# kmaninis/OSVOS-PyTorch

Hardware: NVIDIA H100
Metric: frames/sec at 480x854 fwd-only, batch 1 per GPU (OSVOS.forward -> 5 logit maps) (higher is better)
Workload: dtype bf16x3 (split-bf16 operands, fp32 accumulate)

## Files before the change

include/osvos_b200.h:

```cpp
#ifndef OSVOS_B200_H_
#define OSVOS_B200_H_

#include <stddef.h>
#include <stdint.h>

#ifdef __cplusplus
extern "C" {
#endif

#define OSVOS_B200_VERSION 100

#if defined(__GNUC__)
#define OSVOS_API __attribute__((visibility("default")))
#else
#define OSVOS_API
#endif

enum {
  OSVOS_OK = 0,
  OSVOS_ERR_INVALID_ARGUMENT = 1,
  OSVOS_ERR_CUDA = 2,
  OSVOS_ERR_UNSUPPORTED = 3
};

// ... 30 lines not shown
  const void* x_lo;
  const void* w_packed;
  const float* bias;
  void* y_hi;
  void* y_lo;
  float* y_f32;
  const void* mask_hi;
  const float* proj_w;
  const float* proj_b;
  float* pq;
  void* pool_hi;
  void* pool_lo;
  float* colsum;
  int n, h, w, cin, cout;
  int flags;
} osvos_conv3x3_args;
OSVOS_API int osvos_conv3x3(const osvos_conv3x3_args* args , osvos_stream_t stream);

OSVOS_API int osvos_side_folded_multi(const osvos_conv3x3_args* args , int count, osvos_stream_t stream);

typedef struct {
  const float* side_w;
  const float* side_b;
  const float* proj_w;
  const float* proj_b;
  void* packed;
  float* bias2;
  float* folded_f32;
  int cin;
} osvos_fold_item;
OSVOS_API int osvos_fold_side_weights_multi(const osvos_fold_item* items , int count, osvos_stream_t stream);
OSVOS_API int osvos_conv3x3_simt(const osvos_conv3x3_args* args , osvos_stream_t stream);

typedef struct {
// ... 332 lines not shown
```

osvos_pytorch_b200/_native.py:

```python
import ctypes
import os
from ctypes import (POINTER, Structure, c_char_p, c_double, c_float, c_int, c_int32, c_size_t, c_uint8, c_uint32,
                    c_uint64, c_void_p)

_HERE = os.path.dirname(os.path.abspath(__file__))
LIB_PATH = os.path.join(_HERE, "lib", "libosvos_b200.so")

FLAG_RELU = 1
FLAG_FAST = 2
FLAG_RELU_MASK = 4
FLAG_ACCUMULATE = 8
FLAG_DEFER_FINISH = 16
FLAG_DETERMINISTIC = 32
FLAG_VOID_LABELS = 64
WGRAD_FINISH_MAX = 24


class NativeLibraryError(RuntimeError):
    pass


class Conv3x3Args(Structure):
    _fields_ = [("x_hi", c_void_p), ("x_lo", c_void_p), ("w_packed", c_void_p), ("bias", c_void_p),
                ("y_hi", c_void_p), ("y_lo", c_void_p), ("y_f32", c_void_p), ("mask_hi", c_void_p),
                ("proj_w", c_void_p), ("proj_b", c_void_p), ("pq", c_void_p),
                ("pool_hi", c_void_p), ("pool_lo", c_void_p), ("colsum", c_void_p),
                ("n", c_int), ("h", c_int), ("w", c_int), ("cin", c_int), ("cout", c_int), ("flags", c_int)]


class Stage1Args(Structure):
    _fields_ = [("x", c_void_p), ("w1", c_void_p), ("b1", c_void_p), ("w2_packed", c_void_p), ("b2", c_void_p),
                ("y_hi", c_void_p), ("y_lo", c_void_p), ("pool_hi", c_void_p), ("pool_lo", c_void_p),
                ("n", c_int), ("h", c_int), ("w", c_int)]


class TailFwdArgs(Structure):
    _fields_ = [("pq", c_void_p * 4), ("fuse_bias", c_void_p), ("out", c_void_p * 5), ("label", c_void_p),
                ("sums", c_void_p), ("losses", c_void_p), ("loss_weights", c_float * 5), ("divisor", c_float),
                ("n", c_int), ("h", c_int), ("w", c_int), ("flags", c_int)]


TAIL_SUMS = 15
# ... 2 lines not shown
class TailLossBwdArgs(Structure):
    _fields_ = [("logits", c_void_p * 5), ("label", c_void_p), ("sums", c_void_p), ("upstream", c_void_p),
                ("loss_weights", c_float * 5), ("divisor", c_float), ("dpq", c_void_p * 4), ("fuse_bias_grad", c_void_p),
                ("n", c_int), ("h", c_int), ("w", c_int), ("flags", c_int)]


class WgradArgs(Structure):
    _fields_ = [("x_hi", c_void_p), ("x_lo", c_void_p), ("dz_hi", c_void_p), ("dz_lo", c_void_p), ("dw", c_void_p),
                ("workspace", c_void_p), ("n", c_int), ("h", c_int), ("w", c_int), ("cin", c_int), ("cout", c_int),
                ("dz_channels", c_int), ("flags", c_int)]


class WgradFinishItem(Structure):
    _fields_ = [("workspace", c_void_p), ("dw", c_void_p), ("cout", c_int), ("cin", c_int), ("dz_channels", c_int),
                ("accumulate", c_int), ("scale", c_float)]


class FoldItem(Structure):
    _fields_ = [("side_w", c_void_p), ("side_b", c_void_p), ("proj_w", c_void_p), ("proj_b", c_void_p),
                ("packed", c_void_p), ("bias2", c_void_p), ("folded_f32", c_void_p), ("cin", c_int)]


class SideWgradItem(Structure):
    _fields_ = [("x_hi", c_void_p), ("x_lo", c_void_p), ("dpq", c_void_p), ("g", c_void_p), ("n", c_int), ("h", c_int),
                ("w", c_int), ("c", c_int)]


class SideGradsItem(Structure):
    _fields_ = [("g", c_void_p), ("side_w", c_void_p), ("side_b", c_void_p), ("proj_w", c_void_p),
                ("d_side_w", c_void_p), ("d_side_b", c_void_p), ("d_score_w", c_void_p), ("d_score_b", c_void_p),
# ... 62 lines not shown
SGD_MAX_SEGMENTS = 64

SIGNATURES = {
    "osvos_version": (c_int, []),
    "osvos_last_error": (c_char_p, []),
    "osvos_packed_weight_bytes": (c_size_t, [c_int, c_int]),
    "osvos_pack_conv3x3_weights": (c_int, [c_void_p, c_void_p, c_int, c_int, c_int, c_int, c_void_p]),
    "osvos_nchw_to_act": (c_int, [c_void_p, c_void_p, c_void_p, c_int, c_int, c_int, c_int, c_void_p]),
    "osvos_act_to_nchw": (c_int, [c_void_p, c_void_p, c_void_p, c_int, c_int, c_int, c_int, c_void_p]),
    "osvos_conv_first_fwd": (c_int, [c_void_p, c_void_p, c_void_p, c_void_p, c_void_p, c_int, c_int, c_int, c_int,
                                     c_void_p]),
    "osvos_conv3x3": (c_int, [POINTER(Conv3x3Args), c_void_p]),
    "osvos_stage1_fused": (c_int, [POINTER(Stage1Args), c_void_p]),
    "osvos_set_pdl": (c_int, [c_int]),
    "osvos_side_folded_multi": (c_int, [POINTER(Conv3x3Args), c_int, c_void_p]),
    "osvos_fold_side_weights_multi": (c_int, [POINTER(FoldItem), c_int, c_void_p]),
    "osvos_conv3x3_simt": (c_int, [POINTER(Conv3x3Args), c_void_p]),
    "osvos_maxpool2x2_fwd": (c_int, [c_void_p, c_void_p, c_void_p, c_void_p, c_int, c_int, c_int, c_int, c_void_p]),
    "osvos_tail_fwd": (c_int, [POINTER(TailFwdArgs), c_void_p]),
    "osvos_cbce_fwd_sums": (c_size_t, [c_size_t, c_int]),
    "osvos_cbce_fwd": (c_int, [c_void_p, c_void_p, c_size_t, c_double, c_void_p, c_void_p, c_int, c_void_p]),
    "osvos_cbce_bwd": (c_int, [c_void_p, c_void_p, c_void_p, c_void_p, c_double, c_size_t, c_void_p, c_void_p]),
    "osvos_cbce_bwd_void": (c_int, [c_void_p, c_void_p, c_void_p, c_void_p, c_double, c_size_t, c_void_p, c_void_p]),
    "osvos_wgrad_workspace_bytes": (c_size_t, [c_int, c_int, c_int, c_int, c_int, c_int]),
    "osvos_conv3x3_wgrad": (c_int, [POINTER(WgradArgs), c_void_p]),
    "osvos_wgrad_finish": (c_int, [POINTER(WgradFinishItem), POINTER(c_int), c_int, c_int, c_void_p]),
    "osvos_tail_bwd": (c_int, [POINTER(TailBwdArgs), c_void_p]),
    "osvos_tail_loss_bwd": (c_int, [POINTER(TailLossBwdArgs), c_void_p]),
    "osvos_sum_f32_scratch_bytes": (c_size_t, [c_int]),
    "osvos_sum_f32": (c_int, [c_void_p, c_size_t, c_void_p, c_void_p, c_int, c_void_p]),
# ... 108 lines not shown
```

osvos_pytorch_b200/autograd.py:

```python
import torch

from . import ops


class _OSVOSFunction(torch.autograd.Function):
    @staticmethod
    def forward(ctx, engine, x, objective, *params):
        with ops.no_uninitialized_fill():
            return _OSVOSFunction._forward(ctx, engine, x, objective, *params)

    @staticmethod
    def backward(ctx, *grads):
        with ops.no_uninitialized_fill():
            return _OSVOSFunction._backward(ctx, *grads)

    @staticmethod
    def _forward(ctx, engine, x, objective, *params):
        m = engine.m
        fast = m.precision == "fast"
        general = engine.uses_general_tail()
        ctx.params = params
        ctx.set_materialize_grads(False)
        det = torch.are_deterministic_algorithms_enabled()
        ctx.det = det
        xin = x.detach().contiguous().float()
        n, _, h, w = (int(v) for v in xin.shape)
        acts, pooled = engine._trunk(xin, fast, keep=True)
        feats, pqs = engine._side_outputs([s[-1] for s in acts[1:]], fast)
        if general:
            table = engine._upsampling_table()
            ctx.general = (feats, pqs, table)

            def tail(**kw):
                return ops.tail_general_fwd(feats, pqs, table, m.fuse.bias.detach(), n, h, w, **kw)
        else:
            ctx.general = None

            def tail(**kw):
                return ops.tail_fwd(pqs, m.fuse.bias.detach(), n, h, w, **kw)
        ctx.engine = engine
        ctx.dims = (n, h, w)
        ctx.fast = fast
# ... 252 lines not shown
```

osvos_pytorch_b200/csrc/conv3x3_halo.cu:

```cuda
#include "conv_common.cuh"

namespace osvos {

constexpr int kHaloRows = kTileH + 2;
constexpr int kPitch = kTileW + 2;

template <int BLOCK_N, int PLANES, bool SPLIT>
struct HaloCfg {
  static constexpr int kABoxBytes = kHaloRows * kPitch * 128;
  static constexpr int kAPlaneBytes = (kABoxBytes + 1023) / 1024 * 1024;
  static constexpr int kAStageBytes = PLANES * kAPlaneBytes;
  static constexpr int kAStages = 2;
  static constexpr int kBPlaneBytes = BLOCK_N * 128;
  static constexpr int kBStageBytes = PLANES * kBPlaneBytes;
  static constexpr int kBudget = 225 * 1024 - kAStages * kAStageBytes;
  static constexpr int kBStagesRaw = kBudget / kBStageBytes;
  static constexpr int kBStages = kBStagesRaw > 9 ? 9 : kBStagesRaw;
  static constexpr bool kSplitAcc = SPLIT;
  static_assert(!SPLIT || (PLANES == 2 && BLOCK_N <= 128), "split accumulators need two planes and 2 * BLOCK_N <= 256");
  static constexpr int kAccCols = kSplitAcc ? 2 * BLOCK_N : BLOCK_N;
  static constexpr int kAcc = kAccCols / 2;
  static constexpr int kSmemBytes = kAStages * kAStageBytes + kBStages * kBStageBytes + 1024 + 512;
  static_assert(kBStages >= 2, "weight ring too shallow");
  static_assert(kSmemBytes <= 227 * 1024, "more than the per-CTA shared memory of sm_90");
// ... 167 lines not shown
          if (tap == 8) pending.bar_a = &a_empty[a_stage];
          if (++b_stage == SB) {
            b_stage = 0;
            b_phase ^= 1;
          }
        }
        if (++a_stage == SA) {
          a_stage = 0;
          a_phase ^= 1;
        }
      }
      wgmma_wait<0>();
#pragma unroll
      for (int h = 0; h < kHalves; ++h) wgmma_fence_operands(acc[h]);
      pending.release(leader);
#pragma unroll
      for (int h = 0; h < kHalves; ++h)
        conv_epilogue<BLOCK_N, Cfg::kSplitAcc, LEAN, DET>(p, acc[h], tile, PINGPONG ? h : wg, wl, lane);
    }
  }
}

template <int BLOCK_N, int PLANES, bool LEAN = false, bool DET = false>
static int launch_halo(const osvos_conv3x3_args* a, cudaStream_t stream) {
  constexpr bool kSplit = PLANES == 2 && BLOCK_N <= 128;
  using Cfg = HaloCfg<BLOCK_N, PLANES, kSplit>;
  ConvParams p;
  fill_conv_params(p, a, BLOCK_N);
  const int sms = device_sm_count();
  CUtensorMap mx_hi, mx_lo, mw_hi, mw_lo;
  {
    const uint64_t dims[4] = {(uint64_t)a->cin, (uint64_t)a->w, (uint64_t)a->h, (uint64_t)a->n};
    const uint64_t strides[3] = {(uint64_t)a->cin * 2, (uint64_t)a->w * a->cin * 2,
// ... 8 lines not shown
  }
  int rc = encode_weight_maps(&mw_hi, &mw_lo, a, BLOCK_N);
  if (rc) return rc;
  const int grid = p.total_tiles < sms ? p.total_tiles : sms;
  constexpr bool kCanPingPong = BLOCK_N == 64 || BLOCK_N == 128;
  const bool pingpong = kCanPingPong && p.total_tiles > 2 * sms;
  auto kern = pingpong ? conv3x3_halo_kernel<BLOCK_N, PLANES, kSplit && BLOCK_N == 64, LEAN, kCanPingPong, DET>
                       : conv3x3_halo_kernel<BLOCK_N, PLANES, kSplit, LEAN, false, DET>;
  static uint64_t attr_done[2] = {0, 0};
  OSVOS_CHECK_CUDA(ensure_dynamic_smem(kern, Cfg::kSmemBytes, &attr_done[pingpong]));
  OSVOS_CHECK_CUDA(launch_pdl(kern, dim3(grid), dim3(kConvThreads), Cfg::kSmemBytes, stream, mx_hi, mx_lo,
                              mw_hi, mw_lo, p));
  return OSVOS_OK;
}

template <bool DET>
static int conv3x3_halo_dispatch(const osvos_conv3x3_args* a, cudaStream_t stream) {
  const bool fast = (a->flags & OSVOS_FLAG_FAST) != 0;
  const bool lean = !fast && !(a->flags & OSVOS_FLAG_RELU_MASK) && a->colsum == nullptr && a->y_f32 == nullptr;
  const int m_tiles = ((a->w + kTileW - 1) / kTileW) * ((a->h + kTileH - 1) / kTileH) * a->n;
  const int sms = device_sm_count();
  const long tiles128 = static_cast<long>(m_tiles) * (a->cout / 128);
  const long waves128 = (tiles128 + sms - 1) / sms;
  const long waves256 = (static_cast<long>(m_tiles) * (a->cout / 256) + sms - 1) / sms;
  if (a->cout == 64 || (waves128 == 1 && tiles128 * 5 <= static_cast<long>(sms) * 3)) {
    if (lean) return launch_halo<64, 2, true>(a, stream);
    return fast ? launch_halo<64, 1, false, DET>(a, stream) : launch_halo<64, 2, false, DET>(a, stream);
  }
  if (fast) {
    const bool prefer256 = waves256 * 1100 < waves128 * 700;
    if (a->cout % 256 == 0 && prefer256) return launch_halo<256, 1, false, DET>(a, stream);
    return launch_halo<128, 1, false, DET>(a, stream);
  }
  if (lean) return launch_halo<128, 2, true>(a, stream);
  return launch_halo<128, 2, false, DET>(a, stream);
}

static int check_conv_args(const osvos_conv3x3_args* a) {
  OSVOS_CHECK_ARG(a != nullptr);
  OSVOS_CHECK_ARG(a->n > 0 && a->h > 0 && a->w > 0);
  OSVOS_CHECK_ARG(a->cin >= 64 && a->cin % 64 == 0);
  OSVOS_CHECK_ARG(a->cout == 2 || a->cout == 16 || a->cout == 64 || (a->cout > 0 && a->cout % 128 == 0));
  OSVOS_CHECK_ARG(a->cout != 2 || (a->pq != nullptr && a->y_hi == nullptr && a->y_f32 == nullptr && a->pool_hi == nullptr &&
                                   a->colsum == nullptr && !(a->flags & (OSVOS_FLAG_RELU | OSVOS_FLAG_RELU_MASK))));
  OSVOS_CHECK_ARG(a->cout != 16 || (a->y_hi == nullptr && a->y_lo == nullptr && !(a->flags & OSVOS_FLAG_RELU_MASK)));
  OSVOS_CHECK_ARG(a->x_hi != nullptr && a->w_packed != nullptr);
  OSVOS_CHECK_ARG((a->flags & OSVOS_FLAG_FAST) || a->x_lo != nullptr);
  OSVOS_CHECK_ARG(a->y_hi != nullptr || a->y_f32 != nullptr || a->pq != nullptr || a->pool_hi != nullptr);
  OSVOS_CHECK_ARG(!(a->flags & OSVOS_FLAG_RELU_MASK) || a->mask_hi != nullptr);
  OSVOS_CHECK_ARG(a->pq == nullptr || a->cout == 2 || (a->cout == 16 && a->proj_w != nullptr));
  OSVOS_CHECK_ARG((a->pool_hi == nullptr && a->colsum == nullptr) || a->cout >= 64);
  OSVOS_CHECK_ARG((reinterpret_cast<uintptr_t>(a->x_hi) & 15) == 0);
  OSVOS_CHECK_ARG((reinterpret_cast<uintptr_t>(a->w_packed) & 15) == 0);
  OSVOS_CHECK_ARG((reinterpret_cast<uintptr_t>(a->bias) & 15) == 0);
  OSVOS_CHECK_ARG(!(a->flags & OSVOS_FLAG_DETERMINISTIC) || (reinterpret_cast<uintptr_t>(a->colsum) & 7) == 0);
  if (a->cout >= 64) {
    const uintptr_t bf16_planes = reinterpret_cast<uintptr_t>(a->y_hi) | reinterpret_cast<uintptr_t>(a->y_lo) |
                                  reinterpret_cast<uintptr_t>(a->pool_hi) | reinterpret_cast<uintptr_t>(a->pool_lo) |
                                  reinterpret_cast<uintptr_t>(a->mask_hi);
    OSVOS_CHECK_ARG((bf16_planes & 3) == 0);
    OSVOS_CHECK_ARG((reinterpret_cast<uintptr_t>(a->y_f32) & 7) == 0);
  }
  return OSVOS_OK;
}

}
// ... 16 lines not shown
      order[j] = order[j - 1];
      order[j - 1] = t;
    }
  return side_conv_multi_dispatch(order, count, static_cast<cudaStream_t>(stream_));
}

extern "C" int osvos_conv3x3(const osvos_conv3x3_args* a, osvos_stream_t stream_) {
  int rc = check_conv_args(a);
  if (rc) return rc;
  cudaStream_t stream = static_cast<cudaStream_t>(stream_);
  if (a->cout == 2 || a->cout == 16) return side_conv_dispatch(a, stream);
  if ((a->flags & OSVOS_FLAG_DETERMINISTIC) && a->colsum != nullptr) return conv3x3_halo_dispatch<true>(a, stream);
  return conv3x3_halo_dispatch<false>(a, stream);
}

extern "C" size_t osvos_conv3x3_colsum_rows(int n, int h, int w) {
  if (n <= 0 || h <= 0 || w <= 0) return 0;
  return static_cast<size_t>(n) * ((h + kTileH - 1) / kTileH) * ((w + kTileW - 1) / kTileW) * 8;
}
```

osvos_pytorch_b200/csrc/conv_common.cuh:

```cuda
#pragma once
#include <stdlib.h>

#include "common.cuh"
#include "ptx.cuh"

namespace osvos {

constexpr int kTileW = 8;
constexpr int kTileH = 16;
constexpr int kBlockM = 128;
constexpr int kBlockK = 64;
constexpr int kConvThreads = 384;
constexpr int kABytes = kBlockM * kBlockK * 2;

struct ConvParams {
  const float* bias;
  __nv_bfloat16* y_hi;
  __nv_bfloat16* y_lo;
  float* y_f32;
  const __nv_bfloat16* mask_hi;
  __nv_bfloat16* pool_hi;
  __nv_bfloat16* pool_lo;
  float* colsum;
  int n, h, w, cin, cout;
  int tiles_x, tiles_y, n_blocks, total_tiles, k_chunks;
  int flags;
  int ablate;
};

__device__ __forceinline__ void decode_tile(const ConvParams& p, int tile, int& nb, int& tx, int& ty, int& img) {
  nb = tile % p.n_blocks;
  int m = tile / p.n_blocks;
  tx = m % p.tiles_x;
  m /= p.tiles_x;
  ty = m % p.tiles_y;
  img = m / p.tiles_y;
}

__device__ __forceinline__ uint32_t sw128_offset(int row, int chunk) { return row * 128 + ((chunk ^ (row & 7)) << 4); }

__device__ __forceinline__ void split_pack2(float a, float b, uint32_t& hi, uint32_t& lo) {
  asm("cvt.rn.bf16x2.f32 %0, %1, %2;" : "=r"(hi) : "f"(b), "f"(a));
  const float ra = a - __uint_as_float(hi << 16);
  const float rb = b - __uint_as_float(hi & 0xFFFF0000u);
  asm("cvt.rn.bf16x2.f32 %0, %1, %2;" : "=r"(lo) : "f"(rb), "f"(ra));
}

template <int BLOCK_N, bool SPLIT_ACC, bool LEAN = false, bool DET = false>
__device__ __forceinline__ void conv_epilogue(const ConvParams& p, const float* acc, int tile, int wg, int wl, int lane) {
  if (p.ablate & 16) return;
  int nb, tx, ty, img;
  decode_tile(p, tile, nb, tx, ty, img);
  const int lx = lane >> 2;
  const int x = tx * kTileW + lx;
  const int y0 = ty * kTileH + wg * 8 + wl * 2;
  const bool va = (y0 < p.h) && (x < p.w), vb = (y0 + 1 < p.h) && (x < p.w);
  const bool relu = (p.flags & OSVOS_FLAG_RELU) != 0;
  const bool masked = !LEAN && (p.flags & OSVOS_FLAG_RELU_MASK) != 0;
  const bool store_ok = !(p.ablate & 8);
  const size_t pix[2] = {(static_cast<size_t>(img) * p.h + y0) * p.w + x, (static_cast<size_t>(img) * p.h + y0 + 1) * p.w + x};
  const bool valid[2] = {va, vb};
  const int oh = (p.h + 1) >> 1, ow = (p.w + 1) >> 1;
  const bool pool_writer = va && !(lx & 1) && store_ok;
  const size_t opix = (static_cast<size_t>(img) * oh + (y0 >> 1)) * ow + (x >> 1);
#pragma unroll
  for (int j = 0; j < BLOCK_N / 8; ++j) {
    const int c = 8 * j + 2 * (lane & 3);
    const int ch = nb * BLOCK_N + c;
    const float2 b = p.bias ? __ldg(reinterpret_cast<const float2*>(p.bias + ch)) : make_float2(0.f, 0.f);
    float f[2][2];
#pragma unroll
    for (int h = 0; h < 2; ++h) {
#pragma unroll
      for (int e = 0; e < 2; ++e) {
        float v = e ? b.y : b.x;
        v += acc[4 * j + 2 * h + e];
        if (SPLIT_ACC) v += acc[BLOCK_N / 2 + 4 * j + 2 * h + e];
        f[h][e] = relu ? fmaxf(v, 0.f) : v;
      }
    }
#pragma unroll
    for (int h = 0; h < 2; ++h) {
      if (!LEAN && masked && valid[h]) {
        const uint32_t m = __ldg(reinterpret_cast<const unsigned int*>(p.mask_hi + pix[h] * p.cout + ch));
        if (!(bf16_lo_to_float(m) > 0.f)) f[h][0] = 0.f;
        if (!(bf16_hi_to_float(m) > 0.f)) f[h][1] = 0.f;
      }
      if (valid[h] && store_ok) {
        if (!LEAN && p.y_f32) *reinterpret_cast<float2*>(p.y_f32 + pix[h] * p.cout + ch) = make_float2(f[h][0], f[h][1]);
        if (p.y_hi) {
          uint32_t hi, lo;
          split_pack2(f[h][0], f[h][1], hi, lo);
          *reinterpret_cast<uint32_t*>(p.y_hi + pix[h] * p.cout + ch) = hi;
          if (p.y_lo) *reinterpret_cast<uint32_t*>(p.y_lo + pix[h] * p.cout + ch) = lo;
        }
// ... 18 lines not shown
      }
    }
    if (p.pool_hi) {
      float m0 = fmaxf(va ? f[0][0] : -INFINITY, vb ? f[1][0] : -INFINITY);
      float m1 = fmaxf(va ? f[0][1] : -INFINITY, vb ? f[1][1] : -INFINITY);
      m0 = fmaxf(m0, __shfl_xor_sync(0xffffffffu, m0, 4));
      m1 = fmaxf(m1, __shfl_xor_sync(0xffffffffu, m1, 4));
      if (pool_writer) {
        uint32_t hi, lo;
        split_pack2(m0, m1, hi, lo);
        *reinterpret_cast<uint32_t*>(p.pool_hi + opix * p.cout + ch) = hi;
        if (p.pool_lo) *reinterpret_cast<uint32_t*>(p.pool_lo + opix * p.cout + ch) = lo;
      }
    }
  }
}

constexpr int kStageBoxBytes = 64 * 64 * 2;

struct OutMaps {
  CUtensorMap y_hi, y_lo;
};

__device__ __forceinline__ void conv_epilogue_staged(const ConvParams& p, const OutMaps& maps, const float* acc, int tile,
                                                     int half, int wl, int lane, uint8_t* box, int bar_id, bool leader) {
  if (p.ablate & 16) return;
  int nb, tx, ty, img;
  decode_tile(p, tile, nb, tx, ty, img);
  const int lx = lane >> 2;
  const bool relu = (p.flags & OSVOS_FLAG_RELU) != 0;
// ... 33 lines not shown
      bulk_commit_group();
    }
  }
}


static inline void fill_conv_params(ConvParams& p, const osvos_conv3x3_args* a, int block_n) {
  p.bias = a->bias;
  p.y_hi = static_cast<__nv_bfloat16*>(a->y_hi);
  p.y_lo = static_cast<__nv_bfloat16*>(a->y_lo);
  p.y_f32 = a->y_f32;
  p.mask_hi = static_cast<const __nv_bfloat16*>(a->mask_hi);
  p.pool_hi = static_cast<__nv_bfloat16*>(a->pool_hi);
  p.pool_lo = static_cast<__nv_bfloat16*>(a->pool_lo);
  p.colsum = a->colsum;
  p.n = a->n;
  p.h = a->h;
  p.w = a->w;
  p.cin = a->cin;
  p.cout = a->cout;
  p.tiles_x = (a->w + kTileW - 1) / kTileW;
  p.tiles_y = (a->h + kTileH - 1) / kTileH;
  p.n_blocks = a->cout / block_n;
  p.total_tiles = p.tiles_x * p.tiles_y * a->n * p.n_blocks;
  p.k_chunks = a->cin / kBlockK;
  p.flags = a->flags;
  {
    static int ablate = -1;
    if (ablate < 0) {
      const char* e = getenv("OSVOS_ABLATE");
// ... 44 lines not shown
```

osvos_pytorch_b200/csrc/layout_kernels.cu:

```cuda
#include "common.cuh"

namespace osvos {

int conv_first_tc_launch(const float* x, const float* w_oihw, const float* bias, void* y_hi, void* y_lo, int n, int h,
                         int w, int flags, cudaStream_t stream);

__global__ void pack_weights_kernel(const float* __restrict__ w, __nv_bfloat16* __restrict__ out, int cout, int cin,
                                    int rows, int cols, int colp, int transpose_flip) {
  const size_t plane = static_cast<size_t>(9) * rows * colp;
  for (size_t i = blockIdx.x * static_cast<size_t>(blockDim.x) + threadIdx.x; i < plane;
       i += static_cast<size_t>(gridDim.x) * blockDim.x) {
    const int col = static_cast<int>(i % colp);
    const int row = static_cast<int>((i / colp) % rows);
    const int tap = static_cast<int>(i / (static_cast<size_t>(colp) * rows));
    float v = 0.f;
    if (col < cols) {
      const int co = transpose_flip ? col : row;
      const int ci = transpose_flip ? row : col;
      const int t = transpose_flip ? 8 - tap : tap;
      v = w[(static_cast<size_t>(co) * cin + ci) * 9 + t];
    }
    __nv_bfloat16 hi, lo;
    split_bf16(v, hi, lo);
    out[i] = hi;
// ... 287 lines not shown
                                    int c, osvos_stream_t stream) {
  OSVOS_CHECK_ARG(x_hi != nullptr && y_hi != nullptr && n > 0 && h > 0 && w > 0 && c > 0 && c % 8 == 0);
  OSVOS_CHECK_ARG((x_lo == nullptr) == (y_lo == nullptr));
  const int oh = (h + 1) / 2, ow = (w + 1) / 2;
  const size_t total = static_cast<size_t>(n) * oh * ow * (c / 8);
  maxpool_kernel<<<grid_for(total, 256), 256, 0, static_cast<cudaStream_t>(stream)>>>(
      static_cast<const __nv_bfloat16*>(x_hi), static_cast<const __nv_bfloat16*>(x_lo),
      static_cast<__nv_bfloat16*>(y_hi), static_cast<__nv_bfloat16*>(y_lo), n, h, w, c, oh, ow);
  OSVOS_CHECK_CUDA(cudaGetLastError());
  return OSVOS_OK;
}

extern "C" int osvos_conv3x3_simt(const osvos_conv3x3_args* a, osvos_stream_t stream) {
  OSVOS_CHECK_ARG(a != nullptr && a->x_hi != nullptr && a->w_packed != nullptr);
  OSVOS_CHECK_ARG((a->flags & OSVOS_FLAG_FAST) || a->x_lo != nullptr);
  OSVOS_CHECK_ARG(a->pq == nullptr && a->pool_hi == nullptr && a->colsum == nullptr);
  const size_t total = static_cast<size_t>(a->n) * a->h * a->w * a->cout;
  conv3x3_simt_kernel<<<grid_for(total, 256), 256, 0, static_cast<cudaStream_t>(stream)>>>(
      static_cast<const __nv_bfloat16*>(a->x_hi), static_cast<const __nv_bfloat16*>(a->x_lo),
      static_cast<const __nv_bfloat16*>(a->w_packed), a->bias, static_cast<__nv_bfloat16*>(a->y_hi),
      static_cast<__nv_bfloat16*>(a->y_lo), a->y_f32, static_cast<const __nv_bfloat16*>(a->mask_hi), a->n, a->h, a->w,
      a->cin, a->cout, a->flags);
  OSVOS_CHECK_CUDA(cudaGetLastError());
  return OSVOS_OK;
}

extern "C" int osvos_side_project(const float* feat, const float* proj_w, const float* proj_b, float* pq, int n, int h,
                                  int w, osvos_stream_t stream) {
  OSVOS_CHECK_ARG(feat != nullptr && proj_w != nullptr && pq != nullptr && n > 0 && h > 0 && w > 0);
  const size_t npix = static_cast<size_t>(n) * h * w;
  side_project_kernel<<<grid_for(npix, 256), 256, 0, static_cast<cudaStream_t>(stream)>>>(feat, proj_w, proj_b, pq,
// ... 5 lines not shown
```

osvos_pytorch_b200/csrc/side_conv.cu:

```cuda
#include <string.h>

#include "conv_common.cuh"

namespace osvos {

constexpr int kSideTileW = 8, kSideTileH = 10;
constexpr int kSideHaloW = 10, kSideHaloH = 12;
constexpr int kSideThreads = 384;
constexpr int kSideABox = kSideHaloW * kSideHaloH * 128;
constexpr int kSideAPlane = 128 * 128;

constexpr int kSideMaxScales = 4;
struct SideScale {
  const float* bias;
  float* y_f32;
  const float* proj_w;
  const float* proj_b;
  float* pq;
  int n, h, w, cin;
  int tiles_x, tiles_y, k_chunks;
  int tile_begin;
  int relu;
};
struct SideParams {
// ... 298 lines not shown
  return OSVOS_OK;
}

int side_conv_dispatch(const osvos_conv3x3_args* a, cudaStream_t stream) {
  const osvos_conv3x3_args* one[1] = {a};
  if (a->cout == 2)
    return (a->flags & OSVOS_FLAG_FAST) ? launch_side<1, 2>(one, 1, stream) : launch_side<2, 2>(one, 1, stream);
  return (a->flags & OSVOS_FLAG_FAST) ? launch_side<1, 16>(one, 1, stream) : launch_side<2, 16>(one, 1, stream);
}

int side_conv_multi_dispatch(const osvos_conv3x3_args* const* args, int count, cudaStream_t stream) {
  const bool fast = (args[0]->flags & OSVOS_FLAG_FAST) != 0;
  return fast ? launch_side<1, 2>(args, count, stream) : launch_side<2, 2>(args, count, stream);
}

}
```

osvos_pytorch_b200/engine.py:

```python
import contextlib
import gc
import os

import torch

from . import ops
from .layers.osvos_layers import bilinear_deconv_weight


@contextlib.contextmanager
def no_collection_during_capture():
    gc.collect()
    enabled = gc.isenabled()
    gc.disable()
    try:
        yield
    finally:
        if enabled:
            gc.enable()


class OSVOSEngine:
    def __init__(self, module):
        object.__setattr__(self, "m", module)
# ... 112 lines not shown
                                         out_act=False, out_f32=True, simt=True)
                pq = ops.side_project(feat, self._proj(i), m.score_dsn[i].bias.detach())
            else:
                _, feat, pq = ops.conv3x3(full, self._packed(sp), sp.bias.detach(), 16, relu=False, fast=fast,
                                          out_act=False, out_f32=True, proj_w=self._proj(i),
                                          proj_b=m.score_dsn[i].bias.detach())
            feats.append(feat)
            pqs.append(pq)
        return feats, pqs

    def _side_outputs(self, stage_outs, fast, want_feats=False, simt=False):
        if want_feats or simt or self.uses_general_tail():
            return self._side_features(stage_outs, fast, simt)
        return None, ops.side_folded_multi(stage_outs, self._folded_side_all(), fast=fast)

    def _trunk(self, x, fast, keep, simt=False, fuse_stage1=False):
        convs = self.m.trunk_convs()
        c11, c12 = convs[0]
        acts, pooled = [[]], [None]
        if fuse_stage1:
            full, a = ops.stage1_fused(x, c11.weight.detach().contiguous().float(), c11.bias.detach(),
                                       self._packed(c12), c12.bias.detach(), pool=True, out_act=keep)
        else:
            a = ops.conv_first(x, c11.weight.detach(), c11.bias.detach(), relu=True, fast=fast)
            if keep:
                acts[0].append(a)
            full, a = ops.conv3x3(a, self._packed(c12), c12.bias.detach(), c12.out_channels, relu=True, fast=fast,
                                  pool=True, out_act=keep)
        acts[0].append(full)
        for i in range(1, 5):
            if keep:
                pooled.append(a)
            acts.append([])
            for j, conv in enumerate(convs[i]):
                if j == len(convs[i]) - 1 and i < 4 and not simt:
                    full, a = ops.conv3x3(a, self._packed(conv), conv.bias.detach(), conv.out_channels, relu=True,
                                          fast=fast, pool=True)
                else:
                    a, _, _ = ops.conv3x3(a, self._packed(conv), conv.bias.detach(), conv.out_channels, relu=True,
                                          fast=fast, simt=simt)
                    full = a
                if keep or j == len(convs[i]) - 1:
                    acts[i].append(full)
            if simt and i < 4:
                a = ops.maxpool2x2(full)
        return acts, pooled

    def forward(self, x, fresh_outputs=True):
        if not isinstance(x, torch.Tensor) or x.dim() != 4 or x.size(1) != 3:
            raise ValueError("OSVOS.forward expects a [N, 3, H, W] tensor")
        if not x.is_cuda:
            raise RuntimeError("osvos_pytorch_b200.OSVOS runs on CUDA (sm_90a) only: move the module and the input "
                               "to the GPU.  There is no CPU fallback for the hot path.")
        needs_grad = torch.is_grad_enabled() and (x.requires_grad or any(p.requires_grad for p in self.m.parameters()))
        if x.device != torch.device("cuda", torch.cuda.current_device()):
            with torch.cuda.device(x.device):
                return self.forward(x, fresh_outputs)
        if needs_grad:
            from .autograd import osvos_apply
            return osvos_apply(self, x)
        if self.use_cuda_graph and not torch.cuda.is_current_stream_capturing():
# ... 80 lines not shown
        from . import _native as nat
        lib = nat.load()
        prev = lib.osvos_set_pdl(1)
        try:
            return self._forward_inference(x, simt, return_intermediates)
        finally:
            lib.osvos_set_pdl(prev)

    def _forward_inference(self, x, simt=False, return_intermediates=False):
        m = self.m
        fast = m.precision == "fast"
        general = self.uses_general_tail()
        x = x.detach().contiguous().float()
        n, _, h, w = (int(v) for v in x.shape)
        fuse_stage1 = not fast and not simt and os.environ.get("OSVOS_FUSE_STAGE1", "0") == "1"
        acts, _ = self._trunk(x, fast, keep=return_intermediates, simt=simt, fuse_stage1=fuse_stage1)
        feats, pqs = self._side_outputs([s[-1] for s in acts[1:]], fast, want_feats=return_intermediates, simt=simt)
        if general:
            out, _ = ops.tail_general_fwd(feats, pqs, self._upsampling_table(), m.fuse.bias.detach(), n, h, w)
        else:
            out, _ = ops.tail_fwd(pqs, m.fuse.bias.detach(), n, h, w)
        outs = [out[k] for k in range(5)]
        if not return_intermediates:
            return outs
        inter = {f"stage{i}": s[-1] for i, s in enumerate(acts)}
        for i in range(4):
            inter[f"side{i + 1}"], inter[f"pq{i + 1}"] = feats[i], pqs[i]
        return outs, inter
```

osvos_pytorch_b200/ops.py:

```python
from ctypes import byref, c_void_p

import torch

from . import _native as nat


MEANVAL = (104.00699, 116.66877, 122.67892)

KERNEL_LAUNCHES = [0]


def _stream():
    return torch.cuda.current_stream().cuda_stream


def _count(n=1):
    KERNEL_LAUNCHES[0] += n


class Act:
    __slots__ = ("hi", "lo")

    def __init__(self, hi, lo):
        self.hi = hi
# ... 139 lines not shown
    pqs = []
    for k, (x, f) in enumerate(zip(xs, folded)):
        n, h, w, cin = x.shape
        pq = torch.empty((n, h, w, 2), dtype=torch.float32, device=x.hi.device)
        a = arr[k]
        a.x_hi, a.x_lo = x.hi.data_ptr(), nat.ptr(x.lo)
        a.w_packed, a.bias, a.pq = f[0].data_ptr(), f[1].data_ptr(), pq.data_ptr()
        a.n, a.h, a.w, a.cin, a.cout = n, h, w, cin, 2
        a.flags = nat.FLAG_FAST if fast else 0
        pqs.append(pq)
    _count()
    nat.check(lib.osvos_side_folded_multi(arr, len(xs), _stream()), "osvos_side_folded_multi")
    return pqs


def conv3x3(x, w_packed, bias, cout, relu=False, fast=False, out_act=True, out_f32=False, mask=None,
            proj_w=None, proj_b=None, simt=False, pool=False, colsum=None, deterministic=False):
    lib = nat.load()
    n, h, w, cin = x.shape
    dev = x.hi.device
    y = Act.empty(n, h, w, cout, dev, fast) if out_act else None
    yf = torch.empty((n, h, w, cout), dtype=torch.float32, device=dev) if out_f32 else None
    pq = torch.empty((n, h, w, 2), dtype=torch.float32, device=dev) if proj_w is not None else None
    a = nat.Conv3x3Args()
    a.x_hi, a.x_lo = x.hi.data_ptr(), nat.ptr(x.lo)
    a.w_packed, a.bias = w_packed.data_ptr(), nat.ptr(bias)
    a.y_hi = nat.ptr(y.hi) if y is not None else None
    a.y_lo = nat.ptr(y.lo) if y is not None else None
    a.y_f32 = nat.ptr(yf)
    a.mask_hi = nat.ptr(mask)
    a.proj_w, a.proj_b, a.pq = nat.ptr(proj_w), nat.ptr(proj_b), nat.ptr(pq)
    yp = Act.empty(n, (h + 1) // 2, (w + 1) // 2, cout, dev, fast) if pool else None
    a.pool_hi = nat.ptr(yp.hi) if pool else None
    a.pool_lo = nat.ptr(yp.lo) if pool else None
    rows = None
    if deterministic and colsum is not None:
        nrows = lib.osvos_conv3x3_colsum_rows(n, h, w)
        rows = torch.empty((nrows, cout), dtype=torch.float32, device=dev)
    a.colsum = nat.ptr(rows if rows is not None else colsum)
    a.n, a.h, a.w, a.cin, a.cout = n, h, w, cin, cout
    a.flags = (nat.FLAG_RELU if relu else 0) | (nat.FLAG_FAST if fast else 0) | \
              (nat.FLAG_RELU_MASK if mask is not None else 0) | (nat.FLAG_DETERMINISTIC if rows is not None else 0)
    fn = lib.osvos_conv3x3_simt if simt else lib.osvos_conv3x3
    _count()
    nat.check(fn(byref(a), _stream()), "osvos_conv3x3")
    if rows is not None:
        reduce_rows(rows, colsum, accumulate=True)
    if pool:
        return y, yp
    return y, yf, pq


def maxpool2x2(x):
    lib = nat.load()
    n, h, w, c = x.shape
    y = Act.empty(n, (h + 1) // 2, (w + 1) // 2, c, x.hi.device, x.lo is None)
    _count()
    nat.check(lib.osvos_maxpool2x2_fwd(x.hi.data_ptr(), nat.ptr(x.lo), y.hi.data_ptr(), nat.ptr(y.lo), n, h, w, c,
                                       _stream()), "osvos_maxpool2x2_fwd")
    return y


def side_project(feat, proj_w, proj_b):
    lib = nat.load()
    n, h, w, c = (int(v) for v in feat.shape)
# ... 817 lines not shown
```

Before: 652.5.

## Fuse side-output projection partials into last trunk conv epilogue with gather kernel

Measured after the change: 664.2 (median of 6 runs). 1.8% higher.

```diff
diff --git a/include/osvos_b200.h b/include/osvos_b200.h
--- a/include/osvos_b200.h
+++ b/include/osvos_b200.h
@@ -68,10 +68,20 @@
   float* colsum;
   int n, h, w, cin, cout;
   int flags;
+  const float* side_w;
+  float* side_z;
 } osvos_conv3x3_args;
 OSVOS_API int osvos_conv3x3(const osvos_conv3x3_args* args , osvos_stream_t stream);
+OSVOS_API int osvos_conv3x3_n_blocks(const osvos_conv3x3_args* args );
 
 OSVOS_API int osvos_side_folded_multi(const osvos_conv3x3_args* args , int count, osvos_stream_t stream);
+typedef struct {
+  const float* z;
+  const float* bias2;
+  float* pq;
+  int n, h, w, n_blocks;
+} osvos_side_gather_item;
+OSVOS_API int osvos_side_gather_multi(const osvos_side_gather_item* items , int count, osvos_stream_t stream);
 
 typedef struct {
   const float* side_w;
diff --git a/osvos_pytorch_b200/_native.py b/osvos_pytorch_b200/_native.py
--- a/osvos_pytorch_b200/_native.py
+++ b/osvos_pytorch_b200/_native.py
@@ -25,7 +25,8 @@
                 ("y_hi", c_void_p), ("y_lo", c_void_p), ("y_f32", c_void_p), ("mask_hi", c_void_p),
                 ("proj_w", c_void_p), ("proj_b", c_void_p), ("pq", c_void_p),
                 ("pool_hi", c_void_p), ("pool_lo", c_void_p), ("colsum", c_void_p),
-                ("n", c_int), ("h", c_int), ("w", c_int), ("cin", c_int), ("cout", c_int), ("flags", c_int)]
+                ("n", c_int), ("h", c_int), ("w", c_int), ("cin", c_int), ("cout", c_int), ("flags", c_int),
+                ("side_w", c_void_p), ("side_z", c_void_p)]
 
 
 class Stage1Args(Structure):
@@ -58,6 +59,11 @@
 class WgradFinishItem(Structure):
     _fields_ = [("workspace", c_void_p), ("dw", c_void_p), ("cout", c_int), ("cin", c_int), ("dz_channels", c_int),
                 ("accumulate", c_int), ("scale", c_float)]
+
+
+class SideGatherItem(Structure):
+    _fields_ = [("z", c_void_p), ("bias2", c_void_p), ("pq", c_void_p), ("n", c_int), ("h", c_int), ("w", c_int),
+                ("n_blocks", c_int)]
 
 
 class FoldItem(Structure):
@@ -150,6 +156,8 @@
     "osvos_stage1_fused": (c_int, [POINTER(Stage1Args), c_void_p]),
     "osvos_set_pdl": (c_int, [c_int]),
     "osvos_side_folded_multi": (c_int, [POINTER(Conv3x3Args), c_int, c_void_p]),
+    "osvos_side_gather_multi": (c_int, [POINTER(SideGatherItem), c_int, c_void_p]),
+    "osvos_conv3x3_n_blocks": (c_int, [POINTER(Conv3x3Args)]),
     "osvos_fold_side_weights_multi": (c_int, [POINTER(FoldItem), c_int, c_void_p]),
     "osvos_conv3x3_simt": (c_int, [POINTER(Conv3x3Args), c_void_p]),
     "osvos_maxpool2x2_fwd": (c_int, [c_void_p, c_void_p, c_void_p, c_void_p, c_int, c_int, c_int, c_int, c_void_p]),
diff --git a/osvos_pytorch_b200/autograd.py b/osvos_pytorch_b200/autograd.py
--- a/osvos_pytorch_b200/autograd.py
+++ b/osvos_pytorch_b200/autograd.py
@@ -25,7 +25,7 @@
         ctx.det = det
         xin = x.detach().contiguous().float()
         n, _, h, w = (int(v) for v in xin.shape)
-        acts, pooled = engine._trunk(xin, fast, keep=True)
+        acts, pooled, _ = engine._trunk(xin, fast, keep=True)
         feats, pqs = engine._side_outputs([s[-1] for s in acts[1:]], fast)
         if general:
             table = engine._upsampling_table()
diff --git a/osvos_pytorch_b200/csrc/conv3x3_halo.cu b/osvos_pytorch_b200/csrc/conv3x3_halo.cu
--- a/osvos_pytorch_b200/csrc/conv3x3_halo.cu
+++ b/osvos_pytorch_b200/csrc/conv3x3_halo.cu
@@ -205,9 +205,19 @@
 #pragma unroll
       for (int h = 0; h < kHalves; ++h) wgmma_fence_operands(acc[h]);
       pending.release(leader);
-#pragma unroll
-      for (int h = 0; h < kHalves; ++h)
-        conv_epilogue<BLOCK_N, Cfg::kSplitAcc, LEAN, DET>(p, acc[h], tile, PINGPONG ? h : wg, wl, lane);
+      if (!(p.ablate & 16)) {
+        float fr[kHalves][BLOCK_N / 2];
+#pragma unroll
+        for (int h = 0; h < kHalves; ++h) {
+          conv_epilogue_values<BLOCK_N, Cfg::kSplitAcc>(p, acc[h], tile % p.n_blocks, lane, fr[h]);
+#pragma unroll
+          for (int i = 0; i < BLOCK_N / 2; ++i) asm volatile("" : "+f"(fr[h][i]));
+        }
+        if (p.side_z) conv_side_partials<BLOCK_N, kHalves>(p, fr, tile, PINGPONG ? 0 : wg, wl, lane);
+#pragma unroll
+        for (int h = 0; h < kHalves; ++h)
+          conv_epilogue_store<BLOCK_N, LEAN, DET>(p, fr[h], tile, PINGPONG ? h : wg, wl, lane);
+      }
     }
   }
 }
@@ -246,26 +256,32 @@
   return OSVOS_OK;
 }
 
+static int halo_block_n(const osvos_conv3x3_args* a, int sms) {
+  const bool fast = (a->flags & OSVOS_FLAG_FAST) != 0;
+  const int m_tiles = ((a->w + kTileW - 1) / kTileW) * ((a->h + kTileH - 1) / kTileH) * a->n;
+  const long tiles128 = static_cast<long>(m_tiles) * (a->cout / 128);
+  const long waves128 = (tiles128 + sms - 1) / sms;
+  const long waves256 = (static_cast<long>(m_tiles) * (a->cout / 256) + sms - 1) / sms;
+  if (a->cout == 64 || (waves128 == 1 && tiles128 * 5 <= static_cast<long>(sms) * 3)) return 64;
+  if (fast && a->cout % 256 == 0 && waves256 * 1100 < waves128 * 700) return 256;
+  return 128;
+}
+
 template <bool DET>
 static int conv3x3_halo_dispatch(const osvos_conv3x3_args* a, cudaStream_t stream) {
   const bool fast = (a->flags & OSVOS_FLAG_FAST) != 0;
   const bool lean = !fast && !(a->flags & OSVOS_FLAG_RELU_MASK) && a->colsum == nullptr && a->y_f32 == nullptr;
-  const int m_tiles = ((a->w + kTileW - 1) / kTileW) * ((a->h + kTileH - 1) / kTileH) * a->n;
-  const int sms = device_sm_count();
-  const long tiles128 = static_cast<long>(m_tiles) * (a->cout / 128);
-  const long waves128 = (tiles128 + sms - 1) / sms;
-  const long waves256 = (static_cast<long>(m_tiles) * (a->cout / 256) + sms - 1) / sms;
-  if (a->cout == 64 || (waves128 == 1 && tiles128 * 5 <= static_cast<long>(sms) * 3)) {
-    if (lean) return launch_halo<64, 2, true>(a, stream);
-    return fast ? launch_halo<64, 1, false, DET>(a, stream) : launch_halo<64, 2, false, DET>(a, stream);
-  }
-  if (fast) {
-    const bool prefer256 = waves256 * 1100 < waves128 * 700;
-    if (a->cout % 256 == 0 && prefer256) return launch_halo<256, 1, false, DET>(a, stream);
-    return launch_halo<128, 1, false, DET>(a, stream);
-  }
-  if (lean) return launch_halo<128, 2, true>(a, stream);
-  return launch_halo<128, 2, false, DET>(a, stream);
+  switch (halo_block_n(a, device_sm_count())) {
+    case 64:
+      if (lean) return launch_halo<64, 2, true>(a, stream);
+      return fast ? launch_halo<64, 1, false, DET>(a, stream) : launch_halo<64, 2, false, DET>(a, stream);
+    case 256:
+      return launch_halo<256, 1, false, DET>(a, stream);
+    default:
+      if (fast) return launch_halo<128, 1, false, DET>(a, stream);
+      if (lean) return launch_halo<128, 2, true>(a, stream);
+      return launch_halo<128, 2, false, DET>(a, stream);
+  }
 }
 
 static int check_conv_args(const osvos_conv3x3_args* a) {
@@ -278,10 +294,14 @@
   OSVOS_CHECK_ARG(a->cout != 16 || (a->y_hi == nullptr && a->y_lo == nullptr && !(a->flags & OSVOS_FLAG_RELU_MASK)));
   OSVOS_CHECK_ARG(a->x_hi != nullptr && a->w_packed != nullptr);
   OSVOS_CHECK_ARG((a->flags & OSVOS_FLAG_FAST) || a->x_lo != nullptr);
-  OSVOS_CHECK_ARG(a->y_hi != nullptr || a->y_f32 != nullptr || a->pq != nullptr || a->pool_hi != nullptr);
+  OSVOS_CHECK_ARG(a->y_hi != nullptr || a->y_f32 != nullptr || a->pq != nullptr || a->pool_hi != nullptr ||
+                  a->side_z != nullptr);
   OSVOS_CHECK_ARG(!(a->flags & OSVOS_FLAG_RELU_MASK) || a->mask_hi != nullptr);
   OSVOS_CHECK_ARG(a->pq == nullptr || a->cout == 2 || (a->cout == 16 && a->proj_w != nullptr));
   OSVOS_CHECK_ARG((a->pool_hi == nullptr && a->colsum == nullptr) || a->cout >= 64);
+  OSVOS_CHECK_ARG(a->side_z == nullptr || (a->cout >= 64 && a->side_w != nullptr && a->y_f32 == nullptr &&
+                                           a->colsum == nullptr && !(a->flags & OSVOS_FLAG_RELU_MASK)));
+  OSVOS_CHECK_ARG(((reinterpret_cast<uintptr_t>(a->side_w) & 7) | (reinterpret_cast<uintptr_t>(a->side_z) & 3)) == 0);
   OSVOS_CHECK_ARG((reinterpret_cast<uintptr_t>(a->x_hi) & 15) == 0);
   OSVOS_CHECK_ARG((reinterpret_cast<uintptr_t>(a->w_packed) & 15) == 0);
   OSVOS_CHECK_ARG((reinterpret_cast<uintptr_t>(a->bias) & 15) == 0);
@@ -328,6 +348,12 @@
   return conv3x3_halo_dispatch<false>(a, stream);
 }
 
+extern "C" int osvos_conv3x3_n_blocks(const osvos_conv3x3_args* a) {
+  if (a == nullptr || a->n <= 0 || a->h <= 0 || a->w <= 0 || !(a->cout == 64 || (a->cout > 0 && a->cout % 128 == 0)))
+    return 0;
+  return a->cout / halo_block_n(a, device_sm_count());
+}
+
 extern "C" size_t osvos_conv3x3_colsum_rows(int n, int h, int w) {
   if (n <= 0 || h <= 0 || w <= 0) return 0;
   return static_cast<size_t>(n) * ((h + kTileH - 1) / kTileH) * ((w + kTileW - 1) / kTileW) * 8;
diff --git a/osvos_pytorch_b200/csrc/conv_common.cuh b/osvos_pytorch_b200/csrc/conv_common.cuh
--- a/osvos_pytorch_b200/csrc/conv_common.cuh
+++ b/osvos_pytorch_b200/csrc/conv_common.cuh
@@ -22,6 +22,8 @@
   __nv_bfloat16* pool_hi;
   __nv_bfloat16* pool_lo;
   float* colsum;
+  const float* side_w;
+  float* side_z;
   int n, h, w, cin, cout;
   int tiles_x, tiles_y, n_blocks, total_tiles, k_chunks;
   int flags;
@@ -46,16 +48,76 @@
   asm("cvt.rn.bf16x2.f32 %0, %1, %2;" : "=r"(lo) : "f"(rb), "f"(ra));
 }
 
-template <int BLOCK_N, bool SPLIT_ACC, bool LEAN = false, bool DET = false>
-__device__ __forceinline__ void conv_epilogue(const ConvParams& p, const float* acc, int tile, int wg, int wl, int lane) {
-  if (p.ablate & 16) return;
+template <int BLOCK_N, bool SPLIT_ACC>
+__device__ __forceinline__ void conv_epilogue_values(const ConvParams& p, const float* acc, int nb, int lane, float* fr) {
+  const bool relu = (p.flags & OSVOS_FLAG_RELU) != 0;
+#pragma unroll
+  for (int j = 0; j < BLOCK_N / 8; ++j) {
+    const int ch = nb * BLOCK_N + 8 * j + 2 * (lane & 3);
+    const float2 b = p.bias ? __ldg(reinterpret_cast<const float2*>(p.bias + ch)) : make_float2(0.f, 0.f);
+#pragma unroll
+    for (int h = 0; h < 2; ++h) {
+#pragma unroll
+      for (int e = 0; e < 2; ++e) {
+        float v = e ? b.y : b.x;
+        v += acc[4 * j + 2 * h + e];
+        if (SPLIT_ACC) v += acc[BLOCK_N / 2 + 4 * j + 2 * h + e];
+        fr[4 * j + 2 * h + e] = relu ? fmaxf(v, 0.f) : v;
+      }
+    }
+  }
+}
+
+template <int BLOCK_N, int HALVES>
+__device__ __forceinline__ void conv_side_partials(const ConvParams& p, const float (*fr)[BLOCK_N / 2], int tile, int half0,
+                                                   int wl, int lane) {
+  int nb, tx, ty, img;
+  decode_tile(p, tile, nb, tx, ty, img);
+  const bool b0 = lane & 1, b1 = (lane >> 1) & 1;
+  const int x = tx * kTileW + (lane >> 2);
+  const size_t npix = static_cast<size_t>(p.n) * p.h * p.w;
+  bool store[HALVES];
+  float* dst[HALVES];
+#pragma unroll
+  for (int h = 0; h < HALVES; ++h) {
+    const int y = ty * kTileH + (half0 + h) * 8 + wl * 2 + b0;
+    store[h] = y < p.h && x < p.w && !(p.ablate & 8);
+    dst[h] = p.side_z + (nb * npix + (static_cast<size_t>(img) * p.h + y) * p.w + x) * 18;
+  }
+  const float* wk = p.side_w + nb * BLOCK_N + 2 * (lane & 3);
+  constexpr int kUnroll = (HALVES == 1 && BLOCK_N == 64) ? 2 : 1;
+#pragma unroll kUnroll
+  for (int k = 0; k < 18; ++k, wk += p.cout) {
+    float z[HALVES][2];
+#pragma unroll
+    for (int h = 0; h < HALVES; ++h) z[h][0] = z[h][1] = 0.f;
+#pragma unroll
+    for (int j = 0; j < BLOCK_N / 8; ++j) {
+      const float2 wv = __ldg(reinterpret_cast<const float2*>(wk + 8 * j));
+#pragma unroll
+      for (int h = 0; h < HALVES; ++h) {
+        z[h][0] = fmaf(fr[h][4 * j + 1], wv.y, fmaf(fr[h][4 * j], wv.x, z[h][0]));
+        z[h][1] = fmaf(fr[h][4 * j + 3], wv.y, fmaf(fr[h][4 * j + 2], wv.x, z[h][1]));
+      }
+    }
+#pragma unroll
+    for (int h = 0; h < HALVES; ++h) {
+      float s = (b0 ? z[h][1] : z[h][0]) + __shfl_xor_sync(0xffffffffu, b0 ? z[h][0] : z[h][1], 1);
+      s += __shfl_xor_sync(0xffffffffu, s, 2);
+      if (store[h] && b1 == (k & 1)) dst[h][k] = s;
+    }
+  }
+}
+
+template <int BLOCK_N, bool LEAN = false, bool DET = false>
+__device__ __forceinline__ void conv_epilogue_store(const ConvParams& p, const float* fr, int tile, int wg, int wl,
+                                                    int lane) {
   int nb, tx, ty, img;
   decode_tile(p, tile, nb, tx, ty, img);
   const int lx = lane >> 2;
   const int x = tx * kTileW + lx;
   const int y0 = ty * kTileH + wg * 8 + wl * 2;
   const bool va = (y0 < p.h) && (x < p.w), vb = (y0 + 1 < p.h) && (x < p.w);
-  const bool relu = (p.flags & OSVOS_FLAG_RELU) != 0;
   const bool masked = !LEAN && (p.flags & OSVOS_FLAG_RELU_MASK) != 0;
   const bool store_ok = !(p.ablate & 8);
   const size_t pix[2] = {(static_cast<size_t>(img) * p.h + y0) * p.w + x, (static_cast<size_t>(img) * p.h + y0 + 1) * p.w + x};
@@ -67,18 +129,7 @@
   for (int j = 0; j < BLOCK_N / 8; ++j) {
     const int c = 8 * j + 2 * (lane & 3);
     const int ch = nb * BLOCK_N + c;
-    const float2 b = p.bias ? __ldg(reinterpret_cast<const float2*>(p.bias + ch)) : make_float2(0.f, 0.f);
-    float f[2][2];
-#pragma unroll
-    for (int h = 0; h < 2; ++h) {
-#pragma unroll
-      for (int e = 0; e < 2; ++e) {
-        float v = e ? b.y : b.x;
-        v += acc[4 * j + 2 * h + e];
-        if (SPLIT_ACC) v += acc[BLOCK_N / 2 + 4 * j + 2 * h + e];
-        f[h][e] = relu ? fmaxf(v, 0.f) : v;
-      }
-    }
+    float f[2][2] = {{fr[4 * j], fr[4 * j + 1]}, {fr[4 * j + 2], fr[4 * j + 3]}};
 #pragma unroll
     for (int h = 0; h < 2; ++h) {
       if (!LEAN && masked && valid[h]) {
@@ -127,6 +178,14 @@
       }
     }
   }
+}
+
+template <int BLOCK_N, bool SPLIT_ACC, bool LEAN = false, bool DET = false>
+__device__ __forceinline__ void conv_epilogue(const ConvParams& p, const float* acc, int tile, int wg, int wl, int lane) {
+  if (p.ablate & 16) return;
+  float fr[BLOCK_N / 2];
+  conv_epilogue_values<BLOCK_N, SPLIT_ACC>(p, acc, tile % p.n_blocks, lane, fr);
+  conv_epilogue_store<BLOCK_N, LEAN, DET>(p, fr, tile, wg, wl, lane);
 }
 
 constexpr int kStageBoxBytes = 64 * 64 * 2;
@@ -190,6 +249,8 @@
   p.pool_hi = static_cast<__nv_bfloat16*>(a->pool_hi);
   p.pool_lo = static_cast<__nv_bfloat16*>(a->pool_lo);
   p.colsum = a->colsum;
+  p.side_w = a->side_w;
+  p.side_z = a->side_z;
   p.n = a->n;
   p.h = a->h;
   p.w = a->w;
diff --git a/osvos_pytorch_b200/csrc/layout_kernels.cu b/osvos_pytorch_b200/csrc/layout_kernels.cu
--- a/osvos_pytorch_b200/csrc/layout_kernels.cu
+++ b/osvos_pytorch_b200/csrc/layout_kernels.cu
@@ -325,7 +325,7 @@
 extern "C" int osvos_conv3x3_simt(const osvos_conv3x3_args* a, osvos_stream_t stream) {
   OSVOS_CHECK_ARG(a != nullptr && a->x_hi != nullptr && a->w_packed != nullptr);
   OSVOS_CHECK_ARG((a->flags & OSVOS_FLAG_FAST) || a->x_lo != nullptr);
-  OSVOS_CHECK_ARG(a->pq == nullptr && a->pool_hi == nullptr && a->colsum == nullptr);
+  OSVOS_CHECK_ARG(a->pq == nullptr && a->pool_hi == nullptr && a->colsum == nullptr && a->side_z == nullptr);
   const size_t total = static_cast<size_t>(a->n) * a->h * a->w * a->cout;
   conv3x3_simt_kernel<<<grid_for(total, 256), 256, 0, static_cast<cudaStream_t>(stream)>>>(
       static_cast<const __nv_bfloat16*>(a->x_hi), static_cast<const __nv_bfloat16*>(a->x_lo),
diff --git a/osvos_pytorch_b200/csrc/side_conv.cu b/osvos_pytorch_b200/csrc/side_conv.cu
--- a/osvos_pytorch_b200/csrc/side_conv.cu
+++ b/osvos_pytorch_b200/csrc/side_conv.cu
@@ -336,4 +336,81 @@
   return fast ? launch_side<1, 2>(args, count, stream) : launch_side<2, 2>(args, count, stream);
 }
 
-}
+struct GatherScale {
+  const float* z;
+  const float* bias2;
+  float* pq;
+  int n, h, w, n_blocks;
+  size_t px_begin;
+};
+struct GatherParams {
+  GatherScale sc[kSideMaxScales];
+  int count;
+  size_t total;
+};
+
+__global__ void __launch_bounds__(256) side_gather_kernel(const __grid_constant__ GatherParams p) {
+  pdl_wait();
+  pdl_launch_dependents();
+  for (size_t i = static_cast<size_t>(blockIdx.x) * blockDim.x + threadIdx.x; i < p.total;
+       i += static_cast<size_t>(gridDim.x) * blockDim.x) {
+    int s = 0;
+    while (s + 1 < p.count && i >= p.sc[s + 1].px_begin) ++s;
+    const GatherScale& L = p.sc[s];
+    const size_t local = i - L.px_begin;
+    const int x = static_cast<int>(local % L.w);
+    const size_t t = local / L.w;
+    const int y = static_cast<int>(t % L.h);
+    const size_t row0 = (t / L.h) * L.h;
+    const size_t npix = static_cast<size_t>(L.n) * L.h * L.w;
+    float sp = L.bias2 ? __ldg(L.bias2) : 0.f, sq = L.bias2 ? __ldg(L.bias2 + 1) : 0.f;
+#pragma unroll 4
+    for (int nb = 0; nb < L.n_blocks; ++nb) {
+      const float* zb = L.z + nb * npix * 18;
+#pragma unroll
+      for (int tap = 0; tap < 9; ++tap) {
+        const int yy = y + tap / 3 - 1, xx = x + tap % 3 - 1;
+        if (yy >= 0 && yy < L.h && xx >= 0 && xx < L.w) {
+          const float2 v = __ldg(reinterpret_cast<const float2*>(zb + ((row0 + yy) * L.w + xx) * 18 + 2 * tap));
+          sp += v.x;
+          sq += v.y;
+        }
+      }
+    }
+    *reinterpret_cast<float2*>(L.pq + local * 2) = make_float2(sp, sq);
+  }
+}
+
+}
+
+using namespace osvos;
+
+extern "C" int osvos_side_gather_multi(const osvos_side_gather_item* items, int count, osvos_stream_t stream) {
+  OSVOS_CHECK_ARG(items != nullptr && count > 0 && count <= kSideMaxScales);
+  GatherParams p;
+  memset(&p, 0, sizeof(p));
+  p.count = count;
+  int order[kSideMaxScales];
+  for (int k = 0; k < count; ++k) {
+    OSVOS_CHECK_ARG(items[k].n_blocks > 0);
+    int j = k;
+    for (; j > 0 && items[order[j - 1]].n_blocks < items[k].n_blocks; --j) order[j] = order[j - 1];
+    order[j] = k;
+  }
+  for (int k = 0; k < count; ++k) {
+    const osvos_side_gather_item& it = items[order[k]];
+    OSVOS_CHECK_ARG(it.z != nullptr && it.pq != nullptr && it.n > 0 && it.h > 0 && it.w > 0 && it.n_blocks > 0);
+    OSVOS_CHECK_ARG(((reinterpret_cast<uintptr_t>(it.z) | reinterpret_cast<uintptr_t>(it.pq)) & 7) == 0);
+    GatherScale& L = p.sc[k];
+    L.z = it.z;
+    L.bias2 = it.bias2;
+    L.pq = it.pq;
+    L.n = it.n, L.h = it.h, L.w = it.w, L.n_blocks = it.n_blocks;
+    L.px_begin = p.total;
+    p.total += static_cast<size_t>(it.n) * it.h * it.w;
+  }
+  const size_t blocks = (p.total + 255) / 256;
+  const int grid = static_cast<int>(blocks < 8192 ? blocks : 8192);
+  OSVOS_CHECK_CUDA(launch_pdl(side_gather_kernel, dim3(grid), dim3(256), 0, static_cast<cudaStream_t>(stream), p));
+  return OSVOS_OK;
+}
diff --git a/osvos_pytorch_b200/engine.py b/osvos_pytorch_b200/engine.py
--- a/osvos_pytorch_b200/engine.py
+++ b/osvos_pytorch_b200/engine.py
@@ -150,7 +150,8 @@
             return self._side_features(stage_outs, fast, simt)
         return None, ops.side_folded_multi(stage_outs, self._folded_side_all(), fast=fast)
 
-    def _trunk(self, x, fast, keep, simt=False, fuse_stage1=False):
+    def _trunk(self, x, fast, keep, simt=False, fuse_stage1=False, side=None):
+        assert side is None or not (keep or simt)
         convs = self.m.trunk_convs()
         c11, c12 = convs[0]
         acts, pooled = [[]], [None]
@@ -164,11 +165,18 @@
             full, a = ops.conv3x3(a, self._packed(c12), c12.bias.detach(), c12.out_channels, relu=True, fast=fast,
                                   pool=True, out_act=keep)
         acts[0].append(full)
+        zs = [] if side is not None else None
         for i in range(1, 5):
             if keep:
                 pooled.append(a)
             acts.append([])
             for j, conv in enumerate(convs[i]):
+                if j == len(convs[i]) - 1 and side is not None:
+                    r = ops.conv3x3(a, self._packed(conv), conv.bias.detach(), conv.out_channels, relu=True, fast=fast,
+                                    pool=i < 4, out_act=False, side=side[i - 1])
+                    zs.append((r[-1], a.shape[:3]))
+                    a = r[1] if i < 4 else None
+                    continue
                 if j == len(convs[i]) - 1 and i < 4 and not simt:
                     full, a = ops.conv3x3(a, self._packed(conv), conv.bias.detach(), conv.out_channels, relu=True,
                                           fast=fast, pool=True)
@@ -180,7 +188,7 @@
                     acts[i].append(full)
             if simt and i < 4:
                 a = ops.maxpool2x2(full)
-        return acts, pooled
+        return acts, pooled, zs
 
     def forward(self, x, fresh_outputs=True):
         if not isinstance(x, torch.Tensor) or x.dim() != 4 or x.size(1) != 3:
@@ -291,8 +299,12 @@
         x = x.detach().contiguous().float()
         n, _, h, w = (int(v) for v in x.shape)
         fuse_stage1 = not fast and not simt and os.environ.get("OSVOS_FUSE_STAGE1", "0") == "1"
-        acts, _ = self._trunk(x, fast, keep=return_intermediates, simt=simt, fuse_stage1=fuse_stage1)
-        feats, pqs = self._side_outputs([s[-1] for s in acts[1:]], fast, want_feats=return_intermediates, simt=simt)
+        side = None if (simt or return_intermediates or general) else [f[2] for f in self._folded_side_all()]
+        acts, _, zs = self._trunk(x, fast, keep=return_intermediates, simt=simt, fuse_stage1=fuse_stage1, side=side)
+        if zs is not None:
+            feats, pqs = None, ops.side_gather_multi([z for z, _ in zs], self._folded_side_all(), [s for _, s in zs])
+        else:
+            feats, pqs = self._side_outputs([s[-1] for s in acts[1:]], fast, want_feats=return_intermediates, simt=simt)
         if general:
             out, _ = ops.tail_general_fwd(feats, pqs, self._upsampling_table(), m.fuse.bias.detach(), n, h, w)
         else:
diff --git a/osvos_pytorch_b200/ops.py b/osvos_pytorch_b200/ops.py
--- a/osvos_pytorch_b200/ops.py
+++ b/osvos_pytorch_b200/ops.py
@@ -177,8 +177,23 @@
     return pqs
 
 
+def side_gather_multi(zs, folded, shapes):
+    lib = nat.load()
+    items = (nat.SideGatherItem * len(zs))()
+    pqs = []
+    for k, (z, f, (n, h, w)) in enumerate(zip(zs, folded, shapes)):
+        pq = torch.empty((n, h, w, 2), dtype=torch.float32, device=z.device)
+        it = items[k]
+        it.z, it.bias2, it.pq = z.data_ptr(), f[1].data_ptr(), pq.data_ptr()
+        it.n, it.h, it.w, it.n_blocks = n, h, w, int(z.shape[0])
+        pqs.append(pq)
+    _count()
+    nat.check(lib.osvos_side_gather_multi(items, len(zs), _stream()), "osvos_side_gather_multi")
+    return pqs
+
+
 def conv3x3(x, w_packed, bias, cout, relu=False, fast=False, out_act=True, out_f32=False, mask=None,
-            proj_w=None, proj_b=None, simt=False, pool=False, colsum=None, deterministic=False):
+            proj_w=None, proj_b=None, simt=False, pool=False, colsum=None, deterministic=False, side=None):
     lib = nat.load()
     n, h, w, cin = x.shape
     dev = x.hi.device
@@ -204,14 +219,20 @@
     a.n, a.h, a.w, a.cin, a.cout = n, h, w, cin, cout
     a.flags = (nat.FLAG_RELU if relu else 0) | (nat.FLAG_FAST if fast else 0) | \
               (nat.FLAG_RELU_MASK if mask is not None else 0) | (nat.FLAG_DETERMINISTIC if rows is not None else 0)
+    z = None
+    if side is not None:
+        nblocks = lib.osvos_conv3x3_n_blocks(byref(a))
+        if nblocks <= 0:
+            raise ValueError(f"conv3x3: side partials need cout 64 or a multiple of 128 (cout {cout})")
+        z = torch.empty((nblocks, n * h * w, 18), dtype=torch.float32, device=dev)
+        a.side_w, a.side_z = side.data_ptr(), z.data_ptr()
     fn = lib.osvos_conv3x3_simt if simt else lib.osvos_conv3x3
     _count()
     nat.check(fn(byref(a), _stream()), "osvos_conv3x3")
     if rows is not None:
         reduce_rows(rows, colsum, accumulate=True)
-    if pool:
-        return y, yp
-    return y, yf, pq
+    out = (y, yp) if pool else (y, yf, pq)
+    return out + (z,) if side is not None else out
 
 
 def maxpool2x2(x):
```
